# quanpn90/avsr

Measured on AMD Instinct MI355X. Metric: AV-frames/sec/GPU (fwd+bwd) on 15s clips; WER parity on LRS2 test, higher is better.
Workload: dtype bf16

## Files before the change

avsr_amd/_lib.py:

```python
import ctypes
import os

import torch

_HERE = os.path.dirname(os.path.abspath(__file__))
LIB_PATH = os.environ.get("AVSR_LIB_PATH_AB") or os.path.join(_HERE, "libavsr_hip.so")

AVSR_F32, AVSR_BF16 = 0, 1
ACT_NONE, ACT_GELU, ACT_RELU = 0, 1, 2

_c_p = ctypes.c_void_p
_i64 = ctypes.c_int64
_f = ctypes.c_float
_i = ctypes.c_int


class GemmParams(ctypes.Structure):
    _fields_ = [
        ("M", _i), ("N", _i), ("K", _i), ("batch", _i),
        ("dtype", _i), ("a_kmajor", _i), ("b_kmajor", _i), ("c_f32", _i),
        ("A", _c_p), ("lda", _i64), ("strideA", _i64),
        ("B", _c_p), ("ldb", _i64), ("strideB", _i64),
        ("C", _c_p), ("ldc", _i64), ("strideC", _i64),
        ("alpha", _f), ("beta", _f),
        ("bias", _c_p),
        ("act", _i), ("epi_bwd", _i),
        ("preact", _c_p),
        ("res", _c_p), ("ldr", _i64), ("strideR", _i64),
        ("gate", _c_p),
        ("drop_p", _f),
        ("seed", ctypes.c_uint64),
        ("splitk", _i),
        ("ws", _c_p),
        ("db", _c_p),
        ("db_ws", _c_p),
        ("stamp", _c_p),
        ("skinny_ws", _c_p), ("ln_c1", _c_p), ("ln_eps", ctypes.c_float),
        ("kv_k", _c_p), ("kv_v", _c_p), ("kv_pos", _c_p), ("kv_rows", _i),
        ("slab_cnt", _c_p),
    ]


class ConvParams(ctypes.Structure):
    _fields_ = [
        ("dtype", _i),
        ("nimg", _i), ("hin", _i), ("win", _i), ("cin", _i),
        ("hout", _i), ("wout", _i), ("cout", _i),
        ("kh", _i), ("kw", _i), ("sh", _i), ("sw", _i), ("ph", _i), ("pw", _i),
        ("groups", _i),
        ("ldx", _i64), ("ldy", _i64),
        ("x", _c_p), ("w", _c_p), ("y", _c_p),
        ("dx", _c_p), ("dy", _c_p), ("dw", _c_p),
        ("stats", _c_p),
        ("alpha", _f), ("beta", _f),
# ... 192 lines not shown

class VideoNormParams(ctypes.Structure):
    _fields_ = [
        ("B", _i), ("T", _i), ("H", _i), ("W", _i), ("crop", _i), ("oy", _i), ("ox", _i),
        ("frames", _c_p), ("mean", _f), ("std", _f), ("out", _c_p),
    ]


SYMBOLS = {
    "avsr_version": ([], ctypes.c_char_p),
    "avsr_set_option": ([_i, _i64], _i),
    "avsr_get_option": ([_i], _i64),
    "avsr_gemm": ([ctypes.POINTER(GemmParams), _c_p], _i),
    "avsr_gemm_wgrad_group": ([ctypes.POINTER(GemmParams), _i, _c_p], _i),
    "avsr_gemm_skinny_splits": ([_i, _i, _i], _i),
    "avsr_conv_fwd": ([ctypes.POINTER(ConvParams), _c_p], _i),
    "avsr_conv_bwd_data": ([ctypes.POINTER(ConvParams), _c_p], _i),
    "avsr_conv_bwd_weight": ([ctypes.POINTER(ConvParams), _c_p], _i),
    "avsr_conv_stat_tiles": ([ctypes.POINTER(ConvParams)], _i),
    "avsr_conv_bnr_tiles": ([ctypes.POINTER(ConvParams)], _i),
    "avsr_conv_wgrad_ws": ([ctypes.POINTER(ConvParams)], _i64),
    "avsr_conv_path": ([ctypes.POINTER(ConvParams), _i], _i),
    "avsr_layernorm_fwd": ([ctypes.POINTER(LayerNormParams), _c_p], _i),
    "avsr_layernorm_bwd": ([ctypes.POINTER(LayerNormParams), _c_p], _i),
    "avsr_bn_finalize": ([ctypes.POINTER(BnFinalizeParams), _c_p], _i),
    "avsr_bn_act_fwd": ([ctypes.POINTER(BnActParams), _c_p], _i),
    "avsr_bn_act_bwd_reduce": ([ctypes.POINTER(BnActParams), _c_p], _i),
    "avsr_bn_bwd_apply": ([ctypes.POINTER(BnActParams), _c_p], _i),
    "avsr_stem_pool_fwd": ([ctypes.POINTER(StemPoolParams), _c_p], _i),
    "avsr_stem_pool_bwd_apply": ([ctypes.POINTER(StemPoolParams), _c_p], _i),
# ... 71 lines not shown
            continue
        fn = getattr(lib, name)
        fn.argtypes = argtypes
        fn.restype = restype
    _lib = lib
    return lib


def check(rc, op):
    if rc != 0:
        raise AvsrLibError(f"{op} failed with code {rc}")


OPTIONS = {"gemm_tile": 0, "attn_sq_fwd": 1, "attn_sq_bwd": 2, "wgrad_dual": 3, "conv_192": 4, "conv_s2phase": 5,
           "conv_patch": 6, "conv_wpatch": 7, "stem_pool_2x2": 8,
           "stem_wpatch": 9, "attn_enc_fused": 10}
TILES = ["128", "256", "256x128", "128x256", "128s3", "128w8s3", "pp", "192", "192x256", "192w8s3", "64", "64s4"]
ATTN_PATHS = ["f32", "tiled", "resident", "sq", "enc"]
CONV_PATHS = ["reg", "glds", "patch", "s2", "wpatch", "stem_wpatch"]
CONV_PASSES = ["fwd", "dgrad", "wgrad"]


def set_option(name, value):
    if name == "gemm_tile" and not isinstance(value, int):
        value = 0 if value in (None, "auto") else TILES.index(value) + 1
    lib = load()
    prev = get_option(name)
    check(lib.avsr_set_option(OPTIONS[name], int(value)), f"avsr_set_option({name}, {value})")
    return prev


# ... 16 lines not shown
```

avsr_amd/csrc/gemm.hip:

```cpp
#include "gemm_dense.h"
#include "gemm_pp.h"
#include <type_traits>
#include <utility>

using namespace gemmd;

namespace {

template <typename T, typename OutT, int WM, int WN, bool AK, bool BK>
__global__ __launch_bounds__(NT) void dense_kernel(DenseArgs a) {
  extern __shared__ __attribute__((aligned(16))) char smem[];
  using TL = Tile<T, WM, WN, AK, BK>;
  const int z = blockIdx.z, bz = z / a.splits, sp = z % a.splits;
  const int m0 = blockIdx.y * TL::BM, n0 = blockIdx.x * TL::BN;
  using LA = typename std::conditional<AK, LdDenseK<T, TL::BM>, LdDenseR<T, TL::BM>>::type;
  using LB = typename std::conditional<BK, LdDenseK<T, TL::BN>, LdDenseR<T, TL::BN>>::type;
  LA la; la.p = (const T*)a.A + (int64_t)bz * a.sA; la.ld = a.lda; la.rext = a.M; la.K = a.K;
  LB lb; lb.p = (const T*)a.B + (int64_t)bz * a.sB; lb.ld = a.ldb; lb.rext = a.N; lb.K = a.K;
  const int kbeg = sp * a.kchunk, kend = min(a.K, kbeg + a.kchunk);
  f32x16 acc[2][2];
  mainloop<T, WM, WN>(la, lb, m0, n0, kbeg, kend, acc, smem);
  const Epi e = tile_epi<T, OutT, EV_GENERIC>(a, bz, sp);
  epilogue<T, OutT, WM, WN>(e, m0, n0, acc, smem);
}
// ... 20 lines not shown
  } else {
    using LA = typename std::conditional<AK, gemmg::GDenseK<CF::BM, CF::NW>, gemmg::GDenseR<CF::BM, CF::NW>>::type;
    using LB = typename std::conditional<BK, gemmg::GDenseK<CF::BN, CF::NW>, gemmg::GDenseR<CF::BN, CF::NW>>::type;
    LA la; la.init((const bf16*)a.A + (int64_t)bz * a.sA, a.lda, m0, a.M, kend, wave, lane);
    LB lb; lb.init((const bf16*)a.B + (int64_t)bz * a.sB, a.ldb, n0, a.N, kend, wave, lane);
    gemmg::mainloop_glds<CF>(la, lb, kbeg, nk, acc, smem);
  }
  const Epi e = tile_epi<bf16, OutT, EV>(a, bz, sp);
  gemmg::epilogue_g<bf16, OutT, CF, EV>(e, m0, n0, acc, smem);
  if (a.stamp != nullptr) {
    __syncthreads();
    if (threadIdx.x == 0) atomicMax(a.stamp + 1, (unsigned long long)__builtin_amdgcn_s_memrealtime());
  }
}

template <typename OutT, bool AK, bool BK>
__global__ __launch_bounds__(gemmpp::NTH, 1) void dense_pp_kernel(DenseArgs a, int tiles_m, int tiles_n) {
  extern __shared__ __attribute__((aligned(16))) char smem[];
  const int id = gemmg::xcd_remap(blockIdx.x, gridDim.x);
  int tm, tn, z;
  gemmg::tile_of(id, tiles_m, tiles_n, tm, tn, z);
  const int bz = z / a.splits, sp = z % a.splits;
  const int m0 = tm * gemmpp::BM, n0 = tn * gemmpp::BN;
  const int kbeg = sp * a.kchunk, kend = min(a.K, kbeg + a.kchunk);
  const int lane = threadIdx.x & 63, wave = __builtin_amdgcn_readfirstlane(threadIdx.x >> 6);
  using LA = typename std::conditional<AK, gemmpp::HalfK<64>, gemmpp::HalfR<64>>::type;
  using LB = typename std::conditional<BK, gemmpp::HalfK<32>, gemmpp::HalfR<32>>::type;
  LA la; la.init((const bf16*)a.A + (int64_t)bz * a.sA, a.lda, m0, a.M, kend, wave, lane);
  LB lb; lb.init((const bf16*)a.B + (int64_t)bz * a.sB, a.ldb, n0, a.N, kend, wave, lane);
  f32x4 acc[8][4];
// ... 145 lines not shown
#endif
int tile_cfg(const avsr_gemm_params* p, int splits) {
  const int forced = (int)avsr_opt(AVSR_OPT_GEMM_TILE) - 1;
  if (forced >= 0) return forced;
  const long tiles_z = (long)p->batch * splits;
  const long t128 = (long)((p->M + 127) / 128) * ((p->N + 127) / 128) * tiles_z;
  if (p->a_kmajor) {
    const long t192 = (long)((p->M + 191) / 192) * ((p->N + 127) / 128) * tiles_z;
    const long n128 = (t128 + 255) / 256, n192 = (t192 + 255) / 256;
    if (n192 >= 2 && 3 * n192 * 50 <= 2 * n128 * 51) return AVSR_AB_FWD2;
    if (t192 > 128 && t192 <= 256) return AVSR_AB_ROUND1;
  }
  const long t64 = (long)((p->M + 63) / 64) * ((p->N + 63) / 64) * tiles_z;
  if (t128 < 256 && t64 >= 2 * t128) return (t64 <= 256 && p->K >= 2048) ? AVSR_TILE_64s4 : AVSR_TILE_64;
  return AVSR_TILE_128;
}

template <typename OutT>
int glds_by_layout(const avsr_gemm_params* p, int cfg, const DenseArgs& a, hipStream_t st) {
  if (p->a_kmajor && p->b_kmajor) return launch_cfg<OutT, true, true>(Tiles{}, cfg, a, p->batch, st);
  if (p->a_kmajor) return launch_cfg<OutT, true, false>(Tiles{}, cfg, a, p->batch, st);
  if (p->b_kmajor) return launch_cfg<OutT, false, true>(Tiles{}, cfg, a, p->batch, st);
  return launch_cfg<OutT, false, false>(Tiles{}, cfg, a, p->batch, st);
}

template <typename T, typename OutT, int WM, int WN, bool AK, bool BK>
int launch(const DenseArgs& a, int batch, hipStream_t st) {
  using TL = Tile<T, WM, WN, AK, BK>;
  dim3 grid((a.N + TL::BN - 1) / TL::BN, (a.M + TL::BM - 1) / TL::BM, batch * a.splits);
  hipLaunchKernelGGL((dense_kernel<T, OutT, WM, WN, AK, BK>), grid, dim3(NT), TL::LDS_BYTES, st, a);
// ... 74 lines not shown
  a.kvk = (float*)p->kv_k; a.kvv = (float*)p->kv_v; a.kvpos = p->kv_pos; a.kvrows = p->kv_rows;
  Epi& e = a.e;
  e.M = p->M; e.N = p->N; e.C = p->C; e.ldc = p->ldc;
  e.alpha = p->alpha; e.beta = p->beta; e.bias = p->bias;
  e.act = p->act; e.bwd = p->epi_bwd; e.atomic = splits > 1 && !slab;
  if (slab) {
    e.C = p->ws; e.ldc = p->N; e.alpha = 1.f; e.beta = 0.f;
    a.sSplit = (int64_t)p->M * p->N + AVSR_GEMM_SLAB_PAD; a.sC = (int64_t)splits * a.sSplit;
  }
  e.preact = p->preact; e.res = p->res; e.ldr = p->ldr; e.gate = p->gate;
  e.drop_p = p->drop_p; e.seed = p->seed;
  e.colsum = p->db ? p->db_ws : nullptr;
  return a;
}

extern "C" int avsr_gemm(const avsr_gemm_params* p, void* stream) {
  if (!p) return AVSR_E_ARG;
  if (p->M == 0 || p->N == 0) return 0;
  const int splits = p->splitk > 1 ? p->splitk : 1;
  const bool slab = splits > 1 && p->ws != nullptr;
  const bool glds = glds_ok(p);
  int rc = check_params(p, splits, slab, glds);
  if (rc) return rc;
  const DenseArgs a = dense_args(p, splits, slab);
  hipStream_t st = (hipStream_t)stream;
  int colsum_bm = 0;
  if (!glds && !slab && skinny_ok(p, splits)) return skinny_launch(p, a, st);
  if (glds && wgrad_dual_ok(p, splits, slab)) {
    bool reduced;
    rc = wgrad_dual_launch(p, a, st, &reduced);
    if (reduced) return rc;
  } else if (glds) {
    const int cfg = tile_cfg(p, splits);
    rc = p->c_f32 ? glds_by_layout<float>(p, cfg, a, st) : glds_by_layout<bf16>(p, cfg, a, st);
    if (p->db) colsum_bm = cfg_bm(Tiles{}, cfg, p->a_kmajor != 0);
  } else if (p->dtype == AVSR_F32) rc = by_tile<float, float>(p, a, st);
  else if (p->c_f32) rc = by_tile<bf16, float>(p, a, st);
  else rc = by_tile<bf16, bf16>(p, a, st);
  if (rc) return rc;
  if (colsum_bm) {
    const int tiles = (p->M + colsum_bm - 1) / colsum_bm;
// ... 14 lines not shown
```

avsr_amd/csrc/gemm_glds.h:

```cpp
#pragma once
#include "gemm_core.h"

namespace gemmg {
using namespace gemmcore;

constexpr int GBK = 64;

static __device__ __attribute__((aligned(16))) uint4 g_zero_line[64];

typedef __attribute__((address_space(3))) void lds_void_t;
typedef const __attribute__((address_space(1))) void gbl_void_t;

AVSR_DEV void glds16(const void* src, char* lds_wave_base) {
  __builtin_amdgcn_global_load_lds((gbl_void_t*)src, (lds_void_t*)lds_wave_base, 16, 0, 0);
}

template <int CPR> AVSR_DEV int rswz(int k) {
  return CPR >= 16 ? ((k & 3) | (((k >> 3) & 1) << 2)) << 1 : (((k >> 1) & 1) | (((k >> 3) & 1) << 1)) << 1;
}

template <int R, int NW> struct GDenseK {
  static constexpr bool KMAJ = true;
  static constexpr int SLOTS = R / 8 / NW;
  const bf16* p[SLOTS];
// ... 363 lines not shown
  if (e.colsum) {
    constexpr int CG = BN / 8, RP = 9;
    __syncthreads();
#pragma unroll
    for (int j = 0; j < 8; ++j) st[tid * RP + j] = cs[j];
    __syncthreads();
    for (int t = tid; t < BN; t += CF::NTH) {
      const int g = t >> 3, j = t & 7;
      float s = 0.f;
      for (int k = g; k < CF::NTH; k += CG) s += st[k * RP + j];
      if (n0 + t < e.N) e.colsum[(int64_t)(m0 / CF::BM) * e.N + n0 + t] = s;
    }
  }
}

struct BnrArgs {
  const bf16* h; const bf16* res;
  const float *scale, *shift, *prelu, *mean, *invstd, *scale2, *shift2, *mean2, *invstd2;
  float* ws;
};

template <class CF, int RES>
AVSR_DEV void epilogue_bnr(const Epi& e, const BnrArgs& b, int m0, int n0, f32x4 (&acc)[CF::TM][CF::TN], char* smem) {
  constexpr int BN = CF::BN, LDR = BN + 4, SR = CF::WM * 32, CG = BN / 8, RP = 33, IT = SR * CG / CF::NTH;
  static_assert(CF::NTH % CG == 0 && (SR * CG) % CF::NTH == 0, "a thread's column group must be fixed");
  static_assert(CF::NTH * RP * 4 <= CF::LDS_BYTES, "partials staging exceeds LDS");
  const int tid = threadIdx.x, lane = tid & 63, wave = tid >> 6;
  const int wm = wave / CF::WN, wn = wave % CF::WN;
  float* st = (float*)smem;
  const int lc = (tid % CG) * 8, col = n0 + lc;
// ... 113 lines not shown
```

avsr_amd/csrc/version.hip:

```cpp
#include <atomic>

#include "common.h"

extern "C" const char* avsr_version(void) { return "avsr_hip 0.2.0 gfx950"; }

#ifndef AVSR_AB_ATTN_ENC_FUSED
#define AVSR_AB_ATTN_ENC_FUSED 1
#endif

namespace {
std::atomic<int64_t> g_opt[AVSR_OPT_COUNT] = {{0}, {1}, {0}, {1}, {1}, {1}, {1}, {1}, {1}, {1}, {AVSR_AB_ATTN_ENC_FUSED}};

bool opt_valid(int option, int64_t v) {
  switch (option) {
    case AVSR_OPT_GEMM_TILE: return v >= 0 && v <= AVSR_TILE_COUNT;
    case AVSR_OPT_ATTN_SQ_BWD: return v == 0;
    case AVSR_OPT_ATTN_SQ_FWD:
    case AVSR_OPT_WGRAD_DUAL:
    case AVSR_OPT_CONV_192:
    case AVSR_OPT_CONV_S2PHASE:
    case AVSR_OPT_CONV_PATCH:
    case AVSR_OPT_CONV_WPATCH:
    case AVSR_OPT_STEM_POOL_2X2:
    case AVSR_OPT_STEM_WPATCH:
    case AVSR_OPT_ATTN_ENC_FUSED: return v == 0 || v == 1;
    default: return false;
  }
}
}

int64_t avsr_opt(int option) { return g_opt[option].load(std::memory_order_relaxed); }

extern "C" int avsr_set_option(int option, int64_t value) {
  if (!opt_valid(option, value)) return AVSR_E_ARG;
  g_opt[option].store(value, std::memory_order_relaxed);
  return 0;
}

extern "C" int64_t avsr_get_option(int option) {
  if (option < 0 || option >= AVSR_OPT_COUNT) return -1;
// ... 3 lines not shown
```

avsr_amd/engine.py:

```python
import math
import os
import random

import numpy as np
import torch

from . import ops
from . import _lib as L
from .arena import Arena

GELU, RELU, NONE = L.ACT_GELU, L.ACT_RELU, L.ACT_NONE
_BN_FUSE = True
_DB_FUSE = True
_COLSUM_DEFER = True
_SIDE_BIAS = True
WGRAD_GROUP = False
SIDE_ORDER = "o,f2,f1,c,q"
ATTN_MASK = True
_CTC_SIDE = True
_STEM_DIRECT = True
_LN_EW_FUSE = True
SIDE_STREAM = True
EARLY_NORM = True
OPT_OVERLAP = True
OPT_OVERLAP_BLOCKS = 128
OPT_CLEAR_IN_UPDATE = True


_STEP_STREAMS = {}


def prioritize_step_stream(device):
    if device.type != "cuda":
        return None
# ... 74 lines not shown
            raise ValueError(f"unknown modality_fuse {cfg.modality_fuse!r}")
        self.fuse_add = getattr(cfg, "modality_fuse", "concat") == "add"
        if getattr(cfg, "modality", "av") not in ("av", "audio", "video"):
            raise ValueError(f"unknown modality {cfg.modality!r}")
        self.last_modality = None
        self.force_modality = None
        self.capture = None
        self._pinned = [(None, None)] * 4
        self._pin_next = 0
        self._nbt = None
        self.side = (torch.cuda.Stream(device=self.device)
                     if self.device.type == "cuda" and SIDE_STREAM else None)
        self._side_ev = [torch.cuda.Event() for _ in range(8)] if self.side is not None else []
        self._amask, self._amask_wait = None, False
        self._amask_ev = torch.cuda.Event() if self.side is not None else None
        self._side_i = 0
        self._side_keep = []
        self._side_defer = None
        E = "encoder.encoder.layers"
        groups = []
        for i in range(self.nl):
            a = f"{E}.{i}.attention."
            groups.append([a + "q_proj.weight", a + "k_proj.weight", a + "v_proj.weight"])
            groups.append([a + "q_proj.bias", a + "k_proj.bias", a + "v_proj.bias"])
        for i in range(self.dl):
            s = f"decoder.decoders.{i}.self_attn."
            groups.append([s + "linear_q.weight", s + "linear_k.weight", s + "linear_v.weight"])
            groups.append([s + "linear_q.bias", s + "linear_k.bias", s + "linear_v.bias"])
            c = f"decoder.decoders.{i}.src_attn."
            groups.append([c + "linear_k.weight", c + "linear_v.weight"])
# ... 164 lines not shown
        if self.side is None:
            self.arena.zero_grad()
            return
        g = self.arena.grad
        arena = self.arena
        done = arena.grads_cleared
        arena.grads_cleared = False

        def clear():
            arena.wait_update()
            if not done:
                g.zero_()
        self._on_side(clear, g)
        self.arena.attach_grads(zero=False)
        self.arena.cleared(everything=not done)

    def join_side(self):
        self._flush_side()
        self._side_defer = None
        if self.side is not None:
            torch.cuda.current_stream(self.device).wait_stream(self.side)
            if self._side_keep:
                self._side_keep.clear()

    def _wgrad(self, dy, x, dW, alpha=1.0):
        M, N = dy.shape
        K = x.shape[1]
        splitk = wgrad_splitk(M, N, K)

        def run():
# ... 591 lines not shown
            self._grads_before_video()
            self.video_bwd(ctx["vctx"], dfeat)
        else:
            self._grads_before_video()
        self.join_side()

    def _encoder_bwd_end(self):
        self._grads_before_video()
        self.join_side()

    def _grads_before_video(self):
        if self.pre_video_grads is not None:
            ops.colsum_flush()
            self._on_side(self.pre_video_grads)

    def decoder_fwd(self, enc, bt, train, save, seeds):
        cfg = self.cfg
        B, T, L1 = bt["B"], bt["T"], bt["L1"]
        R, D, H = B * L1, self.dD, self.dH
        klen = None if bt["full"] else bt["lens"]
        sd_e = seeds.next()
        p_d = cfg.dropout_rate if train else 0.0
        p_att = cfg.transformer_attn_dropout_rate if train else 0.0
        y = self._e(R, D)
        self.ensure_pe(L1)
        ops.embed_fwd(bt["ys_in"], self.w("decoder.embed.0.weight"), self._pe[:L1], math.sqrt(D), y, L1,
                      drop_p=p_d, seed=sd_e)
        ctx = {"sd_e": sd_e, "p_d": p_d, "p_att": p_att, "layers": [], "klen": klen, "L1": L1}
        for i in range(self.dl):
            p = f"decoder.decoders.{i}."
            sa, ca, ff = p + "self_attn.", p + "src_attn.", p + "feed_forward."
            n1, m1, r1 = ops.layernorm_fwd(y, self.arena.master(p + "norm1.weight"), self.arena.master(p + "norm1.bias"), 1e-12)
            qkv = ops.linear_fwd(n1, self.arena.span([sa + "linear_q.weight", sa + "linear_k.weight", sa + "linear_v.weight"]),
                                 self.arena.span([sa + "linear_q.bias", sa + "linear_k.bias", sa + "linear_v.bias"], buf="master"))
            o1 = self._e(R, D)
            lse1 = self._e(B, H, L1, dtype=torch.float32)
            s1 = seeds.next()
            ops.attn_fwd(qkv[:, :D], qkv[:, D:2 * D], qkv[:, 2 * D:], o1, lse1, B=B, H=H, Lq=L1, Lk=L1, causal=True,
                         scale=0.125, drop_p=p_att, seed=s1)
            s2 = seeds.next()
            y1 = ops.linear_fwd(o1, self.w(sa + "linear_out.weight"), self.arena.master(sa + "linear_out.bias"), res=y,
                                drop_p=p_d, seed=s2)
            n2, m2, r2 = ops.layernorm_fwd(y1, self.arena.master(p + "norm2.weight"), self.arena.master(p + "norm2.bias"), 1e-12)
            q2 = ops.linear_fwd(n2, self.w(ca + "linear_q.weight"), self.arena.master(ca + "linear_q.bias"))
            kv = ops.linear_fwd(enc, self.arena.span([ca + "linear_k.weight", ca + "linear_v.weight"]),
                                self.arena.span([ca + "linear_k.bias", ca + "linear_v.bias"], buf="master"))
            o2 = self._e(R, D)
            lse2 = self._e(B, H, L1, dtype=torch.float32)
            s3 = seeds.next()
            ops.attn_fwd(q2, kv[:, :D], kv[:, D:], o2, lse2, B=B, H=H, Lq=L1, Lk=T, klen=klen, scale=0.125,
                         drop_p=p_att, seed=s3)
            s4 = seeds.next()
            y2 = ops.linear_fwd(o2, self.w(ca + "linear_out.weight"), self.arena.master(ca + "linear_out.bias"), res=y1,
                                drop_p=p_d, seed=s4)
            n3, m3, r3 = ops.layernorm_fwd(y2, self.arena.master(p + "norm3.weight"), self.arena.master(p + "norm3.bias"), 1e-12)
            h = self._e(R, self.dF)
            s5 = seeds.next()
            a = ops.linear_fwd(n3, self.w(ff + "w_1.weight"), self.arena.master(ff + "w_1.bias"), act=RELU, preact=h,
                               drop_p=p_d, seed=s5)
            s6 = seeds.next()
            y3 = ops.linear_fwd(a, self.w(ff + "w_2.weight"), self.arena.master(ff + "w_2.bias"), res=y2, drop_p=p_d, seed=s6)
# ... 68 lines not shown
                         delta, B=B, H=H, Lq=L1, Lk=T, klen=klen, scale=0.125, drop_p=p_att, seed=lc["s3"],
                         dq=None if dq32 is not None else dq2)
            if dq32 is not None:
                ops.cast(dq32, dq2)
            if live(ca + "linear_q.bias"):
                self._bias_grad(dq2, self.g(ca + "linear_q.bias"))
            if live(ca + "linear_q.weight"):
                self._wgrad(dq2, lc["n2"], self.g(ca + "linear_q.weight"))
            dn2 = ops.linear_dgrad(dq2, self.w(ca + "linear_q.weight"))
            kvw = [ca + "linear_k.weight", ca + "linear_v.weight"]
            if live(ca + "linear_k.bias", ca + "linear_v.bias"):
                self._bias_grad(dkv, self.arena.span([ca + "linear_k.bias", ca + "linear_v.bias"], buf="g"))
            if live(*kvw):
                self._wgrad(dkv, enc, self.arena.span(kvw, buf="g"))
            if denc is not None:
                ops.linear_dgrad(dkv, self.arena.span(kvw), out=denc, beta=1.0)
            dy, g = ln_bwd(dn2, lc["y1"], p + "norm2", lc["m2"], lc["r2"], dy, ew_of(i, "s2", "self_attn.linear_out.bias"))
            if live(sa + "linear_out.weight"):
                self._wgrad(g, lc["o1"], self.g(sa + "linear_out.weight"))
            do1 = ops.linear_dgrad(g, self.w(sa + "linear_out.weight"))
            dqkv = self._e(R, 3 * D)
            dq32 = self._dq32(R, D)
            delta = self._e(B, H, L1, dtype=torch.float32)
            qkv = lc["qkv"]
            ops.attn_bwd(do1, qkv[:, :D], qkv[:, D:2 * D], qkv[:, 2 * D:], lc["o1"], lc["lse1"], dq32, dqkv[:, D:2 * D],
                         dqkv[:, 2 * D:], delta, B=B, H=H, Lq=L1, Lk=L1, causal=True, scale=0.125, drop_p=p_att, seed=lc["s1"],
                         dq=None if dq32 is not None else dqkv[:, :D])
            if dq32 is not None:
                ops.cast(dq32, dqkv[:, :D])
            nb = [sa + "linear_q.bias", sa + "linear_k.bias", sa + "linear_v.bias"]
            nw = [sa + "linear_q.weight", sa + "linear_k.weight", sa + "linear_v.weight"]
            if live(*nb):
                self._bias_grad(dqkv, self.arena.span(nb, buf="g"))
            if live(*nw):
                self._wgrad(dqkv, lc["n1"], self.arena.span(nw, buf="g"))
            dn1 = ops.linear_dgrad(dqkv, self.arena.span(nw))
            dy, g = ln_bwd(dn1, lc["y"], p + "norm1", lc["m1"], lc["r1"], dy,
                           ew_of(i - 1, "s6", "feed_forward.w_2.bias") if i > 0 else None)
        self._side_layer(False)
        if live("decoder.embed.0.weight"):
            ops.embed_bwd(bt["ys_in"], dy, math.sqrt(D), self.g("decoder.embed.0.weight"), L1, drop_p=p_d, seed=ctx["sd_e"])

    def forward(self, videos, audios, video_lengths, labels, train=True, need_grad=True, seed=None, snap=None):
        cfg = self.cfg
        plan = None
        if need_grad:
            snap = snap or self.trainable()
            plan = self._plan(snap)
            need_grad = snap.any
        if train and need_grad and self.before_forward is not None:
            self.before_forward()
        seeds = self.new_seeds(seed)
        bt = self.prepare(videos, audios, video_lengths, labels)
        B, T = bt["B"], bt["T"]
        M = B * T
        modality = self.draw_modality(train) if self.force_modality is None else self.force_modality[0]
# ... 7 lines not shown
        clse = self._e(M, dtype=torch.float32)
        Lmax = bt["ctc_lab"].shape[1]
        S = 2 * Lmax + 1
        alpha = self._e(B, T, S, dtype=torch.float32)
        gamma = self._e(B, T, S, dtype=torch.float32)
        nll = self._e(B, dtype=torch.float32)
        cp = ops.ctc_params(clog, B, T, self.V, bt["ctc_lab"], bt["ctc_len"], bt["lens"], clse, alpha, gamma, nll)

        def ctc_branch():
            if p_c > 0:
                ops.dropout_fwd(enc, xin, p_c, sd_c)
            ops.linear_fwd(xin, self.w("ctc.ctc_lo.weight"), self.arena.master("ctc.ctc_lo.bias"),
                           out=clog[:, :self.V])
            ops.row_lse(clog, self.V, clse)
            ops.ctc_fwd(cp)
        if _CTC_SIDE:
            self._on_side(ctc_branch, enc, xin, clog, clse, alpha, gamma, nll, bt["ctc_lab"], bt["ctc_len"], bt["lens"])
        else:
            ctc_branch()
        dlog, dctx = self.decoder_fwd(enc, bt, train, need_grad and (plan is None or plan.enc or plan.dec), seeds)
        self.join_side()
        R = dlog.shape[0]
        dlse = self._e(R, dtype=torch.float32)
        rloss = self._e(R, dtype=torch.float32)
        rcorr = self._e(R, dtype=torch.int32)
        ops.lsm_fwd(dlog, self.V, bt["ys_out"], cfg.lsm_weight, dlse, rloss, rcorr)
        out4 = self._e(4, dtype=torch.float32)
        ops.loss_finalize(B, nll, rloss, rcorr, cfg.mtlalpha, out4, att_per_token=self.len_norm)
        if self.capture is not None:
            self.capture.update(enc=enc, clog=clog, dlog=dlog, bt=bt)
        ctx = None
        if need_grad:
            ctx = dict(bt=bt, enc=enc, ectx=ectx, xin=xin, p_c=p_c, sd_c=sd_c, clog=clog, cp=cp, dlog=dlog, dctx=dctx,
                       dlse=dlse, snap=snap, plan=plan)
        return out4, ctx
# ... 89 lines not shown
```

avsr_amd/ops.py:

```python
import ctypes
import os

import torch

from . import _lib as L

_DT = {torch.float32: L.AVSR_F32, torch.bfloat16: L.AVSR_BF16}

PROBE = {}

SLAB_PAD = 1088


def slab_ws(batch, splitk, M, N):
    return batch * splitk * (M * N + SLAB_PAD)


def dtype_code(t):
    try:
        return _DT[t.dtype]
    except KeyError:
        raise L.AvsrLibError(f"unsupported dtype {t.dtype}")


# ... 32 lines not shown

_SLAB_CNT = {}
SLAB_CNT = 4096


def _slab_cnt(device):
    key = (_norm_dev(device), L.stream_ptr().value)
    c = _SLAB_CNT.get(key)
    if c is None:
        if torch.cuda.is_current_stream_capturing():
            raise L.AvsrLibError("slab counters first requested inside a graph capture")
        c = _SLAB_CNT[key] = torch.zeros(SLAB_CNT, device=key[0], dtype=torch.int32)
    return c


def reserve_stream_workspaces(device, dec_attn_floats=0):
    assert not torch.cuda.is_current_stream_capturing()
    device = _norm_dev(device)
    _skinny_ws(device)
    _slab_cnt(device)
    key = (device, L.stream_ptr().value)
    ws = _DA_WS.get(key)
    if dec_attn_floats and (ws is None or ws.numel() < dec_attn_floats):
        _DA_WS[key] = torch.empty(dec_attn_floats, device=device, dtype=torch.float32)


def gemm(A, B, C, *, M, N, K, a_kmajor, b_kmajor, lda, ldb, ldc, batch=1,
         strideA=0, strideB=0, strideC=0, alpha=1.0, beta=0.0, bias=None, act=L.ACT_NONE,
         epi_bwd=False, preact=None, res=None, ldr=None, strideR=0, gate=None, drop_p=0.0, seed=0,
         splitk=1, ws=None, db=None, db_ws=None, skinny_split=None, ln_c1=None, ln_eps=0.0, kv=None):
    lib = L.load()
    assert A.is_cuda and B.is_cuda and C.is_cuda
    assert A.dtype == B.dtype, "A/B dtype mismatch"
    dt = dtype_code(A)
    c_f32 = 1 if (C.dtype == torch.float32 and dt == L.AVSR_BF16) else 0
# ... 15 lines not shown
    p.act, p.epi_bwd = act, int(epi_bwd)
    p.preact = None if preact is None else preact.data_ptr()
    p.res = None if res is None else res.data_ptr()
    p.ldr = ldc if ldr is None else ldr
    p.strideR = strideR
    p.gate = None if gate is None else gate.data_ptr()
    p.drop_p, p.seed = float(drop_p), int(seed) & 0xFFFFFFFFFFFFFFFF
    p.splitk = int(splitk)
    if ws is not None:
        assert ws.dtype == torch.float32 and ws.numel() >= slab_ws(batch, splitk, M, N)
        p.ws = ws.data_ptr()
    if (SKINNY_SPLIT if skinny_split is None else skinny_split) and M <= 64 and splitk <= 1:
        p.skinny_ws = _skinny_ws(A.device).data_ptr()
    elif ws is not None and splitk > 1 and SLAB_FUSED_REDUCE:
        p.slab_cnt = _slab_cnt(A.device).data_ptr()
    if ln_c1 is not None:
        assert ln_c1.dtype == torch.float32 and ln_c1.numel() >= N and dt == L.AVSR_F32
        p.ln_c1, p.ln_eps = ln_c1.data_ptr(), float(ln_eps)
    if kv is not None:
        kc, vc, pos, rows = kv
        assert kc.dtype == vc.dtype == torch.float32 and pos.dtype == torch.int32 and dt == L.AVSR_F32
        p.kv_k, p.kv_v, p.kv_pos, p.kv_rows = kc.data_ptr(), vc.data_ptr(), pos.data_ptr(), int(rows)
    if db is not None:
        assert db.dtype == torch.float32 and db.numel() >= N and db_ws is not None and db_ws.dtype == torch.float32
        assert db_ws.numel() >= ((M + 63) // 64) * N
        p.db, p.db_ws = db.data_ptr(), db_ws.data_ptr()
    probe = PROBE.get("gemm")
    if probe is not None and probe["match"](M, N, K, a_kmajor, b_kmajor, dt):
        i = len(probe["events"])
        st = probe["stamps"]
# ... 783 lines not shown
```

include/avsr_hip.h:

```cpp
#ifndef AVSR_HIP_H
#define AVSR_HIP_H

#include <stdint.h>

#ifdef __cplusplus
extern "C" {
#endif

enum { AVSR_F32 = 0, AVSR_BF16 = 1 };
enum { AVSR_ACT_NONE = 0, AVSR_ACT_GELU = 1, AVSR_ACT_RELU = 2 };
enum { AVSR_E_SHAPE = 1001, AVSR_E_ALIGN = 1002, AVSR_E_DTYPE = 1003, AVSR_E_ARG = 1004 };

const char* avsr_version(void);

enum {
  AVSR_OPT_GEMM_TILE = 0,
  AVSR_OPT_ATTN_SQ_FWD = 1,
  AVSR_OPT_ATTN_SQ_BWD = 2,
  AVSR_OPT_WGRAD_DUAL = 3,
  AVSR_OPT_CONV_192 = 4,
  AVSR_OPT_CONV_S2PHASE = 5,
  AVSR_OPT_CONV_PATCH = 6,
  AVSR_OPT_CONV_WPATCH = 7,
  AVSR_OPT_STEM_POOL_2X2 = 8,
  AVSR_OPT_STEM_WPATCH = 9,
  AVSR_OPT_ATTN_ENC_FUSED = 10,
  AVSR_OPT_COUNT = 11
};
enum {
  AVSR_TILE_128 = 0, AVSR_TILE_256 = 1, AVSR_TILE_256x128 = 2, AVSR_TILE_128x256 = 3, AVSR_TILE_128s3 = 4,
  AVSR_TILE_128w8s3 = 5, AVSR_TILE_PP = 6, AVSR_TILE_192 = 7, AVSR_TILE_192x256 = 8, AVSR_TILE_192w8s3 = 9,
  AVSR_TILE_64 = 10, AVSR_TILE_64s4 = 11, AVSR_TILE_COUNT = 12
};
int avsr_set_option(int option, int64_t value);
int64_t avsr_get_option(int option);

typedef struct {
  int M, N, K, batch;
  int dtype;
  int a_kmajor, b_kmajor;
  int c_f32;
  const void* A; int64_t lda, strideA;
// ... 9 lines not shown
  float drop_p;
  uint64_t seed;
  int splitk;
  float* ws;
  float* db;
  float* db_ws;
  unsigned long long* stamp;
  float* skinny_ws;
  const float* ln_c1;
  float ln_eps;
  void* kv_k;
  void* kv_v;
  const int* kv_pos;
  int kv_rows;
  unsigned* slab_cnt;
} avsr_gemm_params;
#define AVSR_GEMM_COLSUM_WS(M, N) ((int64_t)(((M) + 63) / 64) * (N))
#define AVSR_GEMM_SLAB_PAD 1088
#define AVSR_SKINNY_WS (1 << 19)
#define AVSR_SKINNY_CNT 4096
#define AVSR_SLAB_CNT 4096
#define AVSR_SKINNY_WS_BYTES ((int64_t)AVSR_SKINNY_WS * 4 + AVSR_SKINNY_CNT * 4)
#define AVSR_GEMM_SLAB_WS(batch, splitk, M, N) ((int64_t)(batch) * (splitk) * ((int64_t)(M) * (N) + AVSR_GEMM_SLAB_PAD))

int avsr_gemm(const avsr_gemm_params* p, void* stream);
int avsr_gemm_wgrad_group(const avsr_gemm_params* p, int n, void* stream);
int avsr_gemm_skinny_splits(int dtype, int N, int K);

typedef struct {
  int dtype;
  int nimg, hin, win, cin;
  int hout, wout, cout;
  int kh, kw, sh, sw, ph, pw;
  int groups;
  int64_t ldx, ldy;
  const void* x; const void* w; void* y;
  void* dx; const void* dy; float* dw;
  float* stats;
  float alpha, beta;
  int splitk;
// ... 374 lines not shown
```

Baseline: 148,200.

## Add split-K row-split GEMM for few-row shapes and move decoder KV projections to side stream

```diff
diff --git a/avsr_amd/_lib.py b/avsr_amd/_lib.py
--- a/avsr_amd/_lib.py
+++ b/avsr_amd/_lib.py
@@ -38,6 +38,7 @@
         ("skinny_ws", _c_p), ("ln_c1", _c_p), ("ln_eps", ctypes.c_float),
         ("kv_k", _c_p), ("kv_v", _c_p), ("kv_pos", _c_p), ("kv_rows", _i),
         ("slab_cnt", _c_p),
+        ("rs_ws", _c_p),
     ]
 
 
@@ -260,6 +261,7 @@
     "avsr_gemm": ([ctypes.POINTER(GemmParams), _c_p], _i),
     "avsr_gemm_wgrad_group": ([ctypes.POINTER(GemmParams), _i, _c_p], _i),
     "avsr_gemm_skinny_splits": ([_i, _i, _i], _i),
+    "avsr_gemm_row_splits": ([_i, _i, _i, _i], _i),
     "avsr_conv_fwd": ([ctypes.POINTER(ConvParams), _c_p], _i),
     "avsr_conv_bwd_data": ([ctypes.POINTER(ConvParams), _c_p], _i),
     "avsr_conv_bwd_weight": ([ctypes.POINTER(ConvParams), _c_p], _i),
@@ -361,7 +363,7 @@
 
 OPTIONS = {"gemm_tile": 0, "attn_sq_fwd": 1, "attn_sq_bwd": 2, "wgrad_dual": 3, "conv_192": 4, "conv_s2phase": 5,
            "conv_patch": 6, "conv_wpatch": 7, "stem_pool_2x2": 8,
-           "stem_wpatch": 9, "attn_enc_fused": 10}
+           "stem_wpatch": 9, "attn_enc_fused": 10, "gemm_row_splits": 11}
 TILES = ["128", "256", "256x128", "128x256", "128s3", "128w8s3", "pp", "192", "192x256", "192w8s3", "64", "64s4"]
 ATTN_PATHS = ["f32", "tiled", "resident", "sq", "enc"]
 CONV_PATHS = ["reg", "glds", "patch", "s2", "wpatch", "stem_wpatch"]
diff --git a/avsr_amd/csrc/gemm.hip b/avsr_amd/csrc/gemm.hip
--- a/avsr_amd/csrc/gemm.hip
+++ b/avsr_amd/csrc/gemm.hip
@@ -58,6 +58,38 @@
   }
 }
 
+template <typename OutT, bool BK, class CF>
+__global__ __launch_bounds__(CF::NTH, CF::MINB) void dense_rowsplit_kernel(DenseArgs a, int tiles_m, int tiles_n) {
+  extern __shared__ __attribute__((aligned(16))) char smem[];
+  if (a.stamp != nullptr && threadIdx.x == 0) atomicMin(a.stamp, (unsigned long long)__builtin_amdgcn_s_memrealtime());
+  const int id = gemmg::xcd_remap(blockIdx.x, gridDim.x);
+  const int tile = id / a.splits, sp = id - tile * a.splits;
+  int tm, tn, z;
+  gemmg::tile_of(tile, tiles_m, tiles_n, tm, tn, z);
+  const int m0 = tm * CF::BM, n0 = tn * CF::BN;
+  const int kbeg = sp * a.kchunk, kend = min(a.K, kbeg + a.kchunk);
+  const int lane = threadIdx.x & 63, wave = __builtin_amdgcn_readfirstlane(threadIdx.x >> 6);
+  f32x4 acc[CF::TM][CF::TN];
+  const int nk = kend > kbeg ? (kend - kbeg + gemmg::GBK - 1) / gemmg::GBK : 0;
+  if (a.a_bytes) {
+    using LB = typename std::conditional<BK, gemmg::BDenseK<CF::BN, CF::NW>, gemmg::BDenseR<CF::BN, CF::NW>>::type;
+    gemmg::BDenseK<CF::BM, CF::NW> la; la.init((const bf16*)a.A, a.a_bytes, a.lda, m0, a.M, kend, wave, lane);
+    LB lb; lb.init((const bf16*)a.B, a.b_bytes, a.ldb, n0, a.N, kend, wave, lane);
+    gemmg::mainloop_glds<CF>(la, lb, kbeg, nk, acc, smem);
+  } else {
+    using LB = typename std::conditional<BK, gemmg::GDenseK<CF::BN, CF::NW>, gemmg::GDenseR<CF::BN, CF::NW>>::type;
+    gemmg::GDenseK<CF::BM, CF::NW> la; la.init((const bf16*)a.A, a.lda, m0, a.M, kend, wave, lane);
+    LB lb; lb.init((const bf16*)a.B, a.ldb, n0, a.N, kend, wave, lane);
+    gemmg::mainloop_glds<CF>(la, lb, kbeg, nk, acc, smem);
+  }
+  const Epi e = tile_epi<bf16, OutT, EV_GENERIC>(a, 0, 0);
+  gemmg::epilogue_rowsplit<OutT, CF>(e, a.fC, a.cnt, a.splits, tile, sp, m0, n0, acc, smem);
+  if (a.stamp != nullptr) {
+    __syncthreads();
+    if (threadIdx.x == 0) atomicMax(a.stamp + 1, (unsigned long long)__builtin_amdgcn_s_memrealtime());
+  }
+}
+
 template <typename OutT, bool AK, bool BK>
 __global__ __launch_bounds__(gemmpp::NTH, 1) void dense_pp_kernel(DenseArgs a, int tiles_m, int tiles_n) {
   extern __shared__ __attribute__((aligned(16))) char smem[];
@@ -233,6 +265,65 @@
   const long t64 = (long)((p->M + 63) / 64) * ((p->N + 63) / 64) * tiles_z;
   if (t128 < 256 && t64 >= 2 * t128) return (t64 <= 256 && p->K >= 2048) ? AVSR_TILE_64s4 : AVSR_TILE_64;
   return AVSR_TILE_128;
+}
+
+constexpr int ROWSPLIT_TN_MAX = 16, ROWSPLIT_KT_MIN = 48;
+static_assert(AVSR_ROWSPLIT_WS == 16 * 16 * 8 * gemmg::RS_SLAB, "the workspace is sized in slabs");
+
+bool rowsplit_fits(int N, int s) {
+  const int64_t tiles = (int64_t)((AVSR_ROWSPLIT_MAX_M + 63) / 64) * ((N + 63) / 64);
+  return tiles <= AVSR_ROWSPLIT_CNT && tiles * s * gemmg::RS_SLAB <= AVSR_ROWSPLIT_WS;
+}
+
+int rowsplit_rule(int N, int K) {
+  const int tn = (N + 63) / 64, kt = (K + 63) / 64;
+  return (tn <= ROWSPLIT_TN_MAX && kt >= ROWSPLIT_KT_MIN && rowsplit_fits(N, 2)) ? 2 : 1;
+}
+
+int rowsplit_shape(int dtype, int M, int N, int K) {
+  if (dtype != AVSR_BF16 || M < AVSR_ROWSPLIT_MIN_M || M > AVSR_ROWSPLIT_MAX_M || N < 128 || (N % 8) || (K % 8)) return 1;
+  if ((long)((AVSR_ROWSPLIT_MAX_M + 127) / 128) * ((N + 127) / 128) >= 256) return 1;
+  const int opt = (int)avsr_opt(AVSR_OPT_GEMM_ROW_SPLITS);
+  if (opt == 1) return 1;
+  if (opt > 1) return rowsplit_fits(N, opt) ? opt : 1;
+  return rowsplit_rule(N, K);
+}
+
+int rowsplit_of(const avsr_gemm_params* p, int* cfg) {
+  if (!p->rs_ws || p->batch != 1 || p->splitk > 1 || !p->a_kmajor || p->db) return 1;
+  const uintptr_t ptrs = (uintptr_t)p->C | (uintptr_t)p->preact | (uintptr_t)p->res | (uintptr_t)p->gate | (uintptr_t)p->bias;
+  if ((ptrs & 15u) || (p->ldc % 8) || (p->ldr % 8)) return 1;
+  const int s = rowsplit_shape(p->dtype, p->M, p->N, p->K);
+  if (s == 1) return 1;
+  *cfg = tile_cfg(p, 1);
+  if (*cfg != AVSR_TILE_64 && *cfg != AVSR_TILE_64s4) return 1;
+  if (avsr_opt(AVSR_OPT_GEMM_TILE) == 0 && (long)((p->M + 63) / 64) * ((p->N + 63) / 64) * s > 512) *cfg = AVSR_TILE_64;
+  return s;
+}
+
+template <typename OutT, bool BK, class CF>
+int launch_rowsplit_cf(const DenseArgs& a, hipStream_t st) {
+  const int tm = (a.M + CF::BM - 1) / CF::BM, tn = (a.N + CF::BN - 1) / CF::BN;
+  if ((int64_t)tm * tn > AVSR_ROWSPLIT_CNT || (int64_t)tm * tn * a.splits * gemmg::RS_SLAB > AVSR_ROWSPLIT_WS) return AVSR_E_SHAPE;
+  hipLaunchKernelGGL((dense_rowsplit_kernel<OutT, BK, CF>), dim3((unsigned)(tm * tn * a.splits)), dim3(CF::NTH),
+                     CF::LDS_BYTES, st, a, tm, tn);
+  AVSR_CHECK_LAUNCH();
+  return 0;
+}
+
+int launch_rowsplit(const avsr_gemm_params* p, int cfg, int splits, hipStream_t st) {
+  DenseArgs a = dense_args(p, splits, false);
+  a.kchunk = ((p->K + splits - 1) / splits + gemmg::GBK - 1) / gemmg::GBK * gemmg::GBK;
+  a.e.atomic = 0;
+  a.fC = p->rs_ws;
+  a.cnt = (unsigned*)(p->rs_ws + AVSR_ROWSPLIT_WS);
+  const bool s4 = cfg == AVSR_TILE_64s4;
+  if (p->c_f32) {
+    if (p->b_kmajor) return s4 ? launch_rowsplit_cf<float, true, Cfg64s4>(a, st) : launch_rowsplit_cf<float, true, Cfg64>(a, st);
+    return s4 ? launch_rowsplit_cf<float, false, Cfg64s4>(a, st) : launch_rowsplit_cf<float, false, Cfg64>(a, st);
+  }
+  if (p->b_kmajor) return s4 ? launch_rowsplit_cf<bf16, true, Cfg64s4>(a, st) : launch_rowsplit_cf<bf16, true, Cfg64>(a, st);
+  return s4 ? launch_rowsplit_cf<bf16, false, Cfg64s4>(a, st) : launch_rowsplit_cf<bf16, false, Cfg64>(a, st);
 }
 
 template <typename OutT>
@@ -337,6 +428,11 @@
   return a;
 }
 
+extern "C" int avsr_gemm_row_splits(int dtype, int M, int N, int K) {
+  if (M <= 0 || N <= 0 || K <= 0) return 1;
+  return rowsplit_shape(dtype, M, N, K);
+}
+
 extern "C" int avsr_gemm(const avsr_gemm_params* p, void* stream) {
   if (!p) return AVSR_E_ARG;
   if (p->M == 0 || p->N == 0) return 0;
@@ -348,6 +444,7 @@
   const DenseArgs a = dense_args(p, splits, slab);
   hipStream_t st = (hipStream_t)stream;
   int colsum_bm = 0;
+  if (int cfg = 0, rs = rowsplit_of(p, &cfg); rs > 1) return launch_rowsplit(p, cfg, rs, st);
   if (!glds && !slab && skinny_ok(p, splits)) return skinny_launch(p, a, st);
   if (glds && wgrad_dual_ok(p, splits, slab)) {
     bool reduced;
diff --git a/avsr_amd/csrc/gemm_glds.h b/avsr_amd/csrc/gemm_glds.h
--- a/avsr_amd/csrc/gemm_glds.h
+++ b/avsr_amd/csrc/gemm_glds.h
@@ -401,6 +401,85 @@
   }
 }
 
+constexpr int RS_SLAB = 64 * 64 + 32;
+
+template <typename OutT, class CF, int S>
+AVSR_DEV void rowsplit_reduce(const Epi& e, __amdgpu_buffer_rsrc_t rs, int m0, int n0) {
+  constexpr int BN = CF::BN, SR = CF::WM * 32, CGV = BN / 8, IT = SR * CGV / CF::NTH;
+  const int tid = threadIdx.x, lc0 = (tid % CGV) * 8;
+  f32x4 pv[S][IT][2];
+#pragma unroll
+  for (int q = 0; q < S; ++q)
+#pragma unroll
+    for (int it = 0; it < IT; ++it) {
+      const int lr = (tid + it * CF::NTH) / CGV;
+      const uint32_t off = (uint32_t)((q * RS_SLAB + lr * BN + lc0) * 4);
+      pv[q][it][0] = __builtin_bit_cast(f32x4, __builtin_amdgcn_raw_buffer_load_b128(rs, off, 0, 16 ));
+      pv[q][it][1] = __builtin_bit_cast(f32x4, __builtin_amdgcn_raw_buffer_load_b128(rs, off + 16, 0, 16 ));
+    }
+#pragma unroll
+  for (int it = 0; it < IT; ++it) {
+    f32x4 s0 = pv[0][it][0], s1 = pv[0][it][1];
+#pragma unroll
+    for (int q = 1; q < S; ++q) { s0 += pv[q][it][0]; s1 += pv[q][it][1]; }
+    const int lr = (tid + it * CF::NTH) / CGV;
+    const int row = m0 + lr, col = n0 + lc0;
+    if (row < e.M && col < e.N) {
+      float v[8] = {s0[0], s0[1], s0[2], s0[3], s1[0], s1[1], s1[2], s1[3]};
+      epi_vec8<bf16, OutT>(e, row, col, v);
+    }
+  }
+}
+
+template <typename OutT, class CF>
+AVSR_DEV void epilogue_rowsplit(const Epi& e, float* ws, unsigned* cnt, int splits, int tile, int sp, int m0, int n0,
+                                f32x4 (&acc)[CF::TM][CF::TN], char* smem) {
+  constexpr int BN = CF::BN, LDR = BN + 4, SR = CF::WM * 32, CGV = BN / 8, IT = SR * CGV / CF::NTH;
+  static_assert(CF::FM == 1 && SR == CF::BM, "one strip holds the whole tile");
+  static_assert(IT * CF::NTH == SR * CGV && CF::NTH % CGV == 0, "whole vectors per thread");
+  static_assert(SR * BN <= RS_SLAB && RS_SLAB % 4 == 0, "a slab holds one tile, 16-byte aligned");
+  static_assert(SR * LDR * 4 + 16 <= CF::LDS_BYTES, "the arrival flag sits behind the strip");
+  const int tid = threadIdx.x, lane = tid & 63, wave = tid >> 6;
+  const int wm = wave / CF::WN, wn = wave % CF::WN;
+  float* st = (float*)smem;
+  int* last = (int*)(smem + SR * LDR * 4);
+  __syncthreads();
+#pragma unroll
+  for (int h = 0; h < 2; ++h)
+#pragma unroll
+    for (int j = 0; j < CF::TN; ++j)
+#pragma unroll
+      for (int r = 0; r < 4; ++r) {
+        const int lr = wm * 32 + h * 16 + 4 * (lane >> 4) + r;
+        st[lr * LDR + (wn * CF::TN + j) * 16 + (lane & 15)] = acc[h][j][r];
+      }
+  __syncthreads();
+  const __amdgpu_buffer_rsrc_t rs = make_rsrc(ws + (int64_t)tile * splits * RS_SLAB, (uint32_t)(splits * RS_SLAB * 4));
+  const int lc0 = (tid % CGV) * 8;
+#pragma unroll
+  for (int it = 0; it < IT; ++it) {
+    const int lr = (tid + it * CF::NTH) / CGV;
+    const f32x4 v0 = *(const f32x4*)(st + lr * LDR + lc0), v1 = *(const f32x4*)(st + lr * LDR + lc0 + 4);
+    const uint32_t off = (uint32_t)((sp * RS_SLAB + lr * BN + lc0) * 4);
+    __builtin_amdgcn_raw_buffer_store_b128(__builtin_bit_cast(v4i32, v0), rs, off, 0, 16 );
+    __builtin_amdgcn_raw_buffer_store_b128(__builtin_bit_cast(v4i32, v1), rs, off + 16, 0, 16 );
+  }
+  asm volatile("s_waitcnt vmcnt(0)" ::: "memory");
+  __syncthreads();
+  if (tid == 0)
+    *last = __hip_atomic_fetch_add(&cnt[tile], 1u, __ATOMIC_RELAXED, __HIP_MEMORY_SCOPE_AGENT) == (unsigned)splits - 1;
+  __syncthreads();
+  if (!*last) return;
+  switch (splits) {
+    case 2: rowsplit_reduce<OutT, CF, 2>(e, rs, m0, n0); break;
+    case 3: rowsplit_reduce<OutT, CF, 3>(e, rs, m0, n0); break;
+    case 4: rowsplit_reduce<OutT, CF, 4>(e, rs, m0, n0); break;
+    case 6: rowsplit_reduce<OutT, CF, 6>(e, rs, m0, n0); break;
+    default: rowsplit_reduce<OutT, CF, 8>(e, rs, m0, n0); break;
+  }
+  if (tid == 0) __hip_atomic_store(&cnt[tile], 0u, __ATOMIC_RELAXED, __HIP_MEMORY_SCOPE_AGENT);
+}
+
 struct BnrArgs {
   const bf16* h; const bf16* res;
   const float *scale, *shift, *prelu, *mean, *invstd, *scale2, *shift2, *mean2, *invstd2;
diff --git a/avsr_amd/csrc/version.hip b/avsr_amd/csrc/version.hip
--- a/avsr_amd/csrc/version.hip
+++ b/avsr_amd/csrc/version.hip
@@ -9,7 +9,7 @@
 #endif
 
 namespace {
-std::atomic<int64_t> g_opt[AVSR_OPT_COUNT] = {{0}, {1}, {0}, {1}, {1}, {1}, {1}, {1}, {1}, {1}, {AVSR_AB_ATTN_ENC_FUSED}};
+std::atomic<int64_t> g_opt[AVSR_OPT_COUNT] = {{0}, {1}, {0}, {1}, {1}, {1}, {1}, {1}, {1}, {1}, {AVSR_AB_ATTN_ENC_FUSED}, {0}};
 
 bool opt_valid(int option, int64_t v) {
   switch (option) {
@@ -24,6 +24,7 @@
     case AVSR_OPT_STEM_POOL_2X2:
     case AVSR_OPT_STEM_WPATCH:
     case AVSR_OPT_ATTN_ENC_FUSED: return v == 0 || v == 1;
+    case AVSR_OPT_GEMM_ROW_SPLITS: return v >= 0 && v <= 8 && v != 5 && v != 7;
     default: return false;
   }
 }
diff --git a/avsr_amd/engine.py b/avsr_amd/engine.py
--- a/avsr_amd/engine.py
+++ b/avsr_amd/engine.py
@@ -18,6 +18,7 @@
 SIDE_ORDER = "o,f2,f1,c,q"
 ATTN_MASK = True
 _CTC_SIDE = True
+DEC_KV_SIDE = True
 _STEM_DIRECT = True
 _LN_EW_FUSE = True
 SIDE_STREAM = True
@@ -122,6 +123,8 @@
         self._side_ev = [torch.cuda.Event() for _ in range(8)] if self.side is not None else []
         self._amask, self._amask_wait = None, False
         self._amask_ev = torch.cuda.Event() if self.side is not None else None
+        self._kv_ev = torch.cuda.Event() if self.side is not None else None
+        self._denc_ev = torch.cuda.Event() if self.side is not None else None
         self._side_i = 0
         self._side_keep = []
         self._side_defer = None
@@ -316,6 +319,13 @@
         self._on_side(clear, g)
         self.arena.attach_grads(zero=False)
         self.arena.cleared(everything=not done)
+
+    def _on_side_now(self, fn, *keep):
+        q, self._side_defer = self._side_defer, None
+        try:
+            return self._on_side(fn, *keep)
+        finally:
+            self._side_defer = q
 
     def join_side(self):
         self._flush_side()
@@ -937,7 +947,24 @@
             ops.colsum_flush()
             self._on_side(self.pre_video_grads)
 
-    def decoder_fwd(self, enc, bt, train, save, seeds):
+    def _dec_kv(self, i, enc, out=None):
+        ca = f"decoder.decoders.{i}.src_attn."
+        return ops.linear_fwd(enc, self.arena.span([ca + "linear_k.weight", ca + "linear_v.weight"]),
+                              self.arena.span([ca + "linear_k.bias", ca + "linear_v.bias"], buf="master"), out=out)
+
+    def dec_kv_side(self, enc):
+        if not DEC_KV_SIDE or self.side is None or self.dl < 2:
+            return None
+        kvs = [self._e(enc.shape[0], 2 * self.dD) for _ in range(1, self.dl)]
+
+        def run():
+            for i, kv in enumerate(kvs, 1):
+                self._dec_kv(i, enc, out=kv)
+            self._kv_ev.record()
+        self._on_side(run, enc, *kvs)
+        return kvs
+
+    def decoder_fwd(self, enc, bt, train, save, seeds, kv_side=None):
         cfg = self.cfg
         B, T, L1 = bt["B"], bt["T"], bt["L1"]
         R, D, H = B * L1, self.dD, self.dH
@@ -966,8 +993,12 @@
                                 drop_p=p_d, seed=s2)
             n2, m2, r2 = ops.layernorm_fwd(y1, self.arena.master(p + "norm2.weight"), self.arena.master(p + "norm2.bias"), 1e-12)
             q2 = ops.linear_fwd(n2, self.w(ca + "linear_q.weight"), self.arena.master(ca + "linear_q.bias"))
-            kv = ops.linear_fwd(enc, self.arena.span([ca + "linear_k.weight", ca + "linear_v.weight"]),
-                                self.arena.span([ca + "linear_k.bias", ca + "linear_v.bias"], buf="master"))
+            if kv_side is not None and i > 0:
+                if i == 1:
+                    torch.cuda.current_stream(self.device).wait_event(self._kv_ev)
+                kv = kv_side[i - 1]
+            else:
+                kv = self._dec_kv(i, enc)
             o2 = self._e(R, D)
             lse2 = self._e(B, H, L1, dtype=torch.float32)
             s3 = seeds.next()
@@ -1066,7 +1097,13 @@
             if live(*kvw):
                 self._wgrad(dkv, enc, self.arena.span(kvw, buf="g"))
             if denc is not None:
-                ops.linear_dgrad(dkv, self.arena.span(kvw), out=denc, beta=1.0)
+                if DEC_KV_SIDE and self.side is not None:
+                    def dmem(dkv=dkv, w=self.arena.span(kvw)):
+                        ops.linear_dgrad(dkv, w, out=denc, beta=1.0)
+                        self._denc_ev.record()
+                    self._on_side_now(dmem, dkv, denc)
+                else:
+                    ops.linear_dgrad(dkv, self.arena.span(kvw), out=denc, beta=1.0)
             dy, g = ln_bwd(dn2, lc["y1"], p + "norm2", lc["m2"], lc["r2"], dy, ew_of(i, "s2", "self_attn.linear_out.bias"))
             if live(sa + "linear_out.weight"):
                 self._wgrad(g, lc["o1"], self.g(sa + "linear_out.weight"))
@@ -1092,6 +1129,8 @@
         self._side_layer(False)
         if live("decoder.embed.0.weight"):
             ops.embed_bwd(bt["ys_in"], dy, math.sqrt(D), self.g("decoder.embed.0.weight"), L1, drop_p=p_d, seed=ctx["sd_e"])
+        if denc is not None and DEC_KV_SIDE and self.side is not None and self.dl:
+            torch.cuda.current_stream(self.device).wait_event(self._denc_ev)
 
     def forward(self, videos, audios, video_lengths, labels, train=True, need_grad=True, seed=None, snap=None):
         cfg = self.cfg
@@ -1129,11 +1168,13 @@
                            out=clog[:, :self.V])
             ops.row_lse(clog, self.V, clse)
             ops.ctc_fwd(cp)
+        kv_side = self.dec_kv_side(enc)
         if _CTC_SIDE:
             self._on_side(ctc_branch, enc, xin, clog, clse, alpha, gamma, nll, bt["ctc_lab"], bt["ctc_len"], bt["lens"])
         else:
             ctc_branch()
-        dlog, dctx = self.decoder_fwd(enc, bt, train, need_grad and (plan is None or plan.enc or plan.dec), seeds)
+        dlog, dctx = self.decoder_fwd(enc, bt, train, need_grad and (plan is None or plan.enc or plan.dec), seeds,
+                                      kv_side=kv_side)
         self.join_side()
         R = dlog.shape[0]
         dlse = self._e(R, dtype=torch.float32)
diff --git a/avsr_amd/ops.py b/avsr_amd/ops.py
--- a/avsr_amd/ops.py
+++ b/avsr_amd/ops.py
@@ -70,11 +70,36 @@
     return c
 
 
+_ROWSPLIT_WS = {}
+ROWSPLIT_WS = 16 * 16 * 8 * (64 * 64 + 32)
+ROWSPLIT_CNT = 4096
+ROWSPLIT_ROWS = (65, 1024)
+ROW_SPLIT = True
+
+
+def row_splits(M, N, K, dtype=torch.bfloat16):
+    code = L.AVSR_BF16 if dtype == torch.bfloat16 else L.AVSR_F32
+    return int(L.load().avsr_gemm_row_splits(code, int(M), int(N), int(K)))
+
+
+def _rowsplit_ws(device):
+    key = (_norm_dev(device), L.stream_ptr().value)
+    ws = _ROWSPLIT_WS.get(key)
+    if ws is None:
+        if torch.cuda.is_current_stream_capturing():
+            raise L.AvsrLibError("few-row split-K workspace first requested inside a graph capture: call "
+                                 "ops.reserve_stream_workspaces() on the capture stream before capturing")
+        ws = _ROWSPLIT_WS[key] = torch.zeros(ROWSPLIT_WS + ROWSPLIT_CNT, device=key[0], dtype=torch.float32)
+    return ws
+
+
 def reserve_stream_workspaces(device, dec_attn_floats=0):
     assert not torch.cuda.is_current_stream_capturing()
     device = _norm_dev(device)
     _skinny_ws(device)
     _slab_cnt(device)
+    if ROW_SPLIT:
+        _rowsplit_ws(device)
     key = (device, L.stream_ptr().value)
     ws = _DA_WS.get(key)
     if dec_attn_floats and (ws is None or ws.numel() < dec_attn_floats):
@@ -120,6 +145,9 @@
         p.skinny_ws = _skinny_ws(A.device).data_ptr()
     elif ws is not None and splitk > 1 and SLAB_FUSED_REDUCE:
         p.slab_cnt = _slab_cnt(A.device).data_ptr()
+    elif (ROW_SPLIT and ROWSPLIT_ROWS[0] <= M <= ROWSPLIT_ROWS[1] and dt == L.AVSR_BF16 and a_kmajor and batch == 1
+          and splitk <= 1 and db is None):
+        p.rs_ws = _rowsplit_ws(A.device).data_ptr()
     if ln_c1 is not None:
         assert ln_c1.dtype == torch.float32 and ln_c1.numel() >= N and dt == L.AVSR_F32
         p.ln_c1, p.ln_eps = ln_c1.data_ptr(), float(ln_eps)
diff --git a/include/avsr_hip.h b/include/avsr_hip.h
--- a/include/avsr_hip.h
+++ b/include/avsr_hip.h
@@ -25,7 +25,8 @@
   AVSR_OPT_STEM_POOL_2X2 = 8,
   AVSR_OPT_STEM_WPATCH = 9,
   AVSR_OPT_ATTN_ENC_FUSED = 10,
-  AVSR_OPT_COUNT = 11
+  AVSR_OPT_GEMM_ROW_SPLITS = 11,
+  AVSR_OPT_COUNT = 12
 };
 enum {
   AVSR_TILE_128 = 0, AVSR_TILE_256 = 1, AVSR_TILE_256x128 = 2, AVSR_TILE_128x256 = 3, AVSR_TILE_128s3 = 4,
@@ -65,16 +66,23 @@
   const int* kv_pos;
   int kv_rows;
   unsigned* slab_cnt;
+  float* rs_ws;
 } avsr_gemm_params;
 #define AVSR_GEMM_COLSUM_WS(M, N) ((int64_t)(((M) + 63) / 64) * (N))
 #define AVSR_GEMM_SLAB_PAD 1088
 #define AVSR_SKINNY_WS (1 << 19)
 #define AVSR_SKINNY_CNT 4096
 #define AVSR_SLAB_CNT 4096
+#define AVSR_ROWSPLIT_MIN_M 65
+#define AVSR_ROWSPLIT_MAX_M 1024
+#define AVSR_ROWSPLIT_WS (16 * 16 * 8 * (64 * 64 + 32))
+#define AVSR_ROWSPLIT_CNT 4096
+#define AVSR_ROWSPLIT_WS_BYTES ((int64_t)AVSR_ROWSPLIT_WS * 4 + AVSR_ROWSPLIT_CNT * 4)
 #define AVSR_SKINNY_WS_BYTES ((int64_t)AVSR_SKINNY_WS * 4 + AVSR_SKINNY_CNT * 4)
 #define AVSR_GEMM_SLAB_WS(batch, splitk, M, N) ((int64_t)(batch) * (splitk) * ((int64_t)(M) * (N) + AVSR_GEMM_SLAB_PAD))
 
 int avsr_gemm(const avsr_gemm_params* p, void* stream);
+int avsr_gemm_row_splits(int dtype, int M, int N, int K);
 int avsr_gemm_wgrad_group(const avsr_gemm_params* p, int n, void* stream);
 int avsr_gemm_skinny_splits(int dtype, int N, int K);
 
```

Result: no change. 149,000, median of 6 (+0.5%).
